# 54rt1n/shardmerge

Hardware: NVIDIA B200
Metric: merged_params_per_sec (higher is better)
Workload: dtype f32

## Files before the change

### shardmerge_b200/csrc/kernels_fft.cu

```cuda
#include <cstdarg>
#include <mutex>
#include "fft_bodies.cuh"
#include "sm_internal.h"

using namespace smfft;

static thread_local char g_err[512] = "";
void sm_set_error(const char* fmt, ...) {
  va_list ap; va_start(ap, fmt); vsnprintf(g_err, sizeof(g_err), fmt, ap); va_end(ap);
}
extern "C" const char* sm_last_error(void) { return g_err; }
extern "C" int sm_version(void) { return 100; }

struct DeviceExec {
  __device__ __forceinline__ int nthreads() const { return (int)blockDim.x; }
  __device__ __forceinline__ int tid_begin() const { return (int)threadIdx.x; }
  __device__ __forceinline__ int tid_end() const { return (int)threadIdx.x + 1; }
  __device__ __forceinline__ void sync() const { __syncthreads(); }
};

extern __shared__ __align__(128) float2 g_dyn_smem[];

__device__ __forceinline__ double warp_sum(double v) {
#pragma unroll
// ... 875 lines not shown
__device__ __forceinline__ void epilogue_store_eo_fast(const RowInvArgs& a, float scale, uint2 bb, uint2* out64, float4* of, int m, pf va,
                                                       pf vb, float& bad) {
  const pf n = pf_bcast(a.inv_n);
  const pf x0 = vb * n, x1 = va * n;
  float y00 = __fmul_rn(pf_lo(x0), scale), y01 = __fmul_rn(pf_hi(x0), scale), y10 = __fmul_rn(pf_lo(x1), scale), y11 = __fmul_rn(pf_hi(x1), scale);
  if (a.out_mode == 0) {
    y00 = __fadd_rn(bf16_bits_to_f32(bb.x & 0xffffu), y00); y10 = __fadd_rn(bits_f32(bb.x & 0xffff0000u), y10);
    y01 = __fadd_rn(bf16_bits_to_f32(bb.y & 0xffffu), y01); y11 = __fadd_rn(bits_f32(bb.y & 0xffff0000u), y11);
    out64[m] = make_uint2(pack_bf16x2_rne(y00, y10), pack_bf16x2_rne(y01, y11));
  } else {
    of[m] = make_float4(y00, y10, y01, y11);
  }
  bad = fmax3_nan(fmax3_nan(bad, fabsf(y00), fabsf(y01)), fabsf(y10), fabsf(y11));
}

__device__ __forceinline__ void epilogue_store_eo(const RowInvArgs& a, float scale, uint2 bb, uint2* out64, float4* of, int m, pf va, pf vb);
struct RowTangleStagedEO {
  const float* re; const float* im; const cf* twC; int H;
  __device__ __forceinline__ void tangle(int k, float& ore, float& oim) const {
    float xr = re[k], xi = im[k], mr = re[2 * H - k], mi = im[2 * H - k];
    if (k == 0) { xi = 0.f; mi = 0.f; }
    const float Ar = xr + mr, Ai = xi - mi, Br = xr - mr, Bi = xi + mi;
    const cf w = ldg_cf(twC + k);
    const float br = Br * w.x + Bi * w.y, bi = Bi * w.x - Br * w.y;
    ore = Ai + br; oim = Ar - bi;
  }
  __device__ __forceinline__ void load(int n, pf& ore, pf& oim) const {
    float u1r, u1i, u2r, u2i;
    tangle(n, u1r, u1i);
    tangle(n + H, u2r, u2i);
    float dr = u1r - u2r, di = u1i - u2i;
    const cf w = ldg_cf(twC + 2 * n);
    cmul(dr, di, w.x, w.y);
    ore = pf_make(u1r + u2r, dr); oim = pf_make(u1i + u2i, di);
  }
};

template <int R1, int R2, int R3, int T, bool kEO>
__global__ void __launch_bounds__(T, 3) k_row2_inv(int R, int C, int P, const __grid_constant__ RowInvArgs a,
                                                   const cf* __restrict__ twC, const cf* __restrict__ twQ, int work_bytes) {
  sm_pdl_enter();
  constexpr int CH = R1 * R2 * R3;
  constexpr int S3 = CH / R3;
  constexpr int kRows = kEO ? 1 : 2;
  constexpr int kTw = kEO ? 4 : 2;
  static_assert(CH / R1 == T && CH / R2 == T && S3 == 2 * T, "k_row2_inv: one butterfly per thread in stages 1-2, two in stage 3");
  __shared__ uint64_t full;
  RowSmem2 sm{reinterpret_cast<ulonglong2*>(g_dyn_smem)};
  char* st_re = reinterpret_cast<char*>(g_dyn_smem) + work_bytes;
  const uint32_t plane_bytes = 4u * (uint32_t)P * kRows;
  char* st_im = st_re + plane_bytes;
  const int tid = threadIdx.x;
  const int npairs = kEO ? R : (R >> 1);
  if (tid == 0) { mbar_init(&full, 1); mbar_fence_init(); }
  __syncthreads();
  const float* im_plane = (a.sel != nullptr && *a.sel != 0) ? a.im_alt : a.im;
  auto prefetch = [&](int pair) {
    if (tid == 0 && pair < npairs) {
      mbar_expect_tx(&full, 2u * plane_bytes);
      bulk_g2s(st_re, a.re + (size_t)pair * kRows * P, plane_bytes, &full);
      bulk_g2s(st_im, im_plane + (size_t)pair * kRows * P, plane_bytes, &full);
    }
  };
  prefetch((int)blockIdx.x);
  const float scale = a.scale_ptr ? *a.scale_ptr : a.scale_host;
  uint32_t phase = 0;
  const int p2 = tid / R1, q2 = tid - p2 * R1;
  const int obase2 = q2 + R1 * R2 * p2, tstep2 = R1 * p2 * kTw;
  for (int pair = blockIdx.x; pair < npairs; pair += gridDim.x) {
    {
      float wr[R1], wi[R1];
      quad_twiddles<R1>(twQ, tid, wr, wi, kEO ? 2 : 1);
      constexpr int Nr = CH / R1;
      pf re[R1], im[R1];
      if constexpr (kEO) {
        mbar_wait(&full, phase); phase ^= 1u;
        RowTangleStagedEO src{reinterpret_cast<const float*>(st_re), reinterpret_cast<const float*>(st_im), twC, CH};
#pragma unroll
        for (int j = 0; j < R1; ++j) src.load(tid + j * Nr, re[j], im[j]);
      } else {
        cf wt[R1];
#pragma unroll
        for (int j = 0; j < R1; ++j) wt[j] = ldg_cf(twC + tid + j * Nr);
        mbar_wait(&full, phase); phase ^= 1u;
        RowTangleStaged2 src{reinterpret_cast<const float*>(st_re), reinterpret_cast<const float*>(st_im), P, CH};
#pragma unroll
        for (int j = 0; j < R1; ++j) src.load(tid + j * Nr, wt[j], re[j], im[j]);
      }
      Dft<R1>::run(re, im);
      sm.store(R1 * tid, re[0], im[0]);
#pragma unroll
      for (int k = 1; k < R1; ++k) {
        pf xr = re[k], xi = im[k];
        cmul(xr, xi, wr[k], wi[k]);
        sm.store(R1 * tid + k, xr, xi);
      }
    }
    __syncthreads();
    prefetch(pair + (int)gridDim.x);
    {
      cf w[R2];
#pragma unroll
      for (int k = 1; k < R2; ++k) w[k] = ldg_cf(twC + tstep2 * k);
      pf re[R2], im[R2];
      constexpr int Nr = CH / R2;
#pragma unroll
      for (int j = 0; j < R2; ++j) sm.load(tid + j * Nr, re[j], im[j]);
      __syncthreads();
      Dft<R2>::run(re, im);
      sm.store(obase2, re[0], im[0]);
#pragma unroll
      for (int k = 1; k < R2; ++k) {
        pf xr = re[k], xi = im[k];
        cmul(xr, xi, w[k].x, w[k].y);
        sm.store(obase2 + k * R1, xr, xi);
      }
    }
    __syncthreads();
    if constexpr (kEO) {
      const uint2* base64 = reinterpret_cast<const uint2*>(a.base + (size_t)pair * C);
      uint2* out64 = a.out_mode == 0 ? reinterpret_cast<uint2*>(a.out_bf16 + (size_t)pair * C) : nullptr;
      float4* of = a.out_mode != 0 ? reinterpret_cast<float4*>(a.out_f32 + (size_t)pair * C) : nullptr;
#pragma unroll
      for (int h = 0; h < 2; ++h) {
        const int b = tid + h * T;
        uint2 bb[R3];
#pragma unroll
        for (int k = 0; k < R3; ++k) bb[k] = a.out_mode == 0 ? __ldg(base64 + b + k * S3) : make_uint2(0u, 0u);
        pf re[R3], im[R3];
#pragma unroll
        for (int j = 0; j < R3; ++j) sm.load(b + j * S3, re[j], im[j]);
        if (h == 1) __syncthreads();
        Dft<R3>::run(re, im);
        float bad = 0.f;
#pragma unroll
        for (int k = 0; k < R3; ++k) epilogue_store_eo_fast(a, scale, bb[k], out64, of, b + k * S3, re[k], im[k], bad);
        if (not_finite(bad)) {
#pragma unroll
          for (int k = 0; k < R3; ++k) epilogue_store_eo(a, scale, bb[k], out64, of, b + k * S3, re[k], im[k]);
        }
      }
    } else {
      const size_t row0 = (size_t)pair * 2;
      const uint32_t* base0 = reinterpret_cast<const uint32_t*>(a.base + row0 * C);
      const uint32_t* base1 = base0 + C / 2;
      uint32_t* out0 = a.out_mode == 0 ? reinterpret_cast<uint32_t*>(a.out_bf16 + row0 * C) : nullptr;
      uint32_t* out1 = out0 + C / 2;
      float* of0 = a.out_mode != 0 ? a.out_f32 + row0 * C : nullptr;
      float* of1 = of0 + C;
#pragma unroll
      for (int h = 0; h < 2; ++h) {
        const int b = tid + h * T;
        uint32_t bb0[R3], bb1[R3];
#pragma unroll
        for (int k = 0; k < R3; ++k) {
          bb0[k] = a.out_mode == 0 ? ldg_u32(base0 + b + k * S3) : 0u;
          bb1[k] = a.out_mode == 0 ? ldg_u32(base1 + b + k * S3) : 0u;
        }
        pf re[R3], im[R3];
#pragma unroll
        for (int j = 0; j < R3; ++j) sm.load(b + j * S3, re[j], im[j]);
        if (h == 1) __syncthreads();
        Dft<R3>::run(re, im);
        float bad = 0.f;
#pragma unroll
        for (int k = 0; k < R3; ++k) epilogue_store2_fast(a, scale, bb0[k], bb1[k], out0, out1, of0, of1, b + k * S3, re[k], im[k], bad);
        if (not_finite(bad)) {
#pragma unroll
          for (int k = 0; k < R3; ++k) epilogue_store2(a, scale, bb0[k], bb1[k], out0, out1, of0, of1, b + k * S3, re[k], im[k]);
        }
      }
    }
  }
}

struct RowTangleGlobal2 {
  const float* re; const float* im; const cf* twC; int P; int Ch;
  __device__ __forceinline__ void load(int k, pf& ore, pf& oim) const {
    pf xr = pf_make(ldg_f32(re + k), ldg_f32(re + P + k)), xi = pf_make(ldg_f32(im + k), ldg_f32(im + P + k));
    pf mr = pf_make(ldg_f32(re + Ch - k), ldg_f32(re + P + Ch - k)), mi = pf_make(ldg_f32(im + Ch - k), ldg_f32(im + P + Ch - k));
    const cf w = ldg_cf(twC + k);
    if (k == 0) { xi = pf_make(0.f, 0.f); mi = xi; }
    const pf Ar = xr + mr, Ai = xi - mi, Br = xr - mr, Bi = xi + mi;
    const pf wx = pf_bcast(w.x), wy = pf_bcast(w.y);
    const pf br = pf_fma(Br, wx, Bi * wy);
    const pf bi = pf_fma(Bi, wx, zero_of(Br) - Br * wy);
    const pf zr = Ar - bi, zi = Ai + br;
    ore = zi; oim = zr;
  }
};

template <int R1, int R2, int R3, int R4, int T, int kCtas>
__global__ void __launch_bounds__(T, kCtas) k_row2_inv4(int R, int C, int P, const __grid_constant__ RowInvArgs a,
                                                    const cf* __restrict__ twC, const cf* __restrict__ twQ) {
  sm_pdl_enter();
  constexpr int CH = R1 * R2 * R3 * R4;
  constexpr int NB1 = CH / R1, NB2 = CH / R2, NB3 = CH / R3, S4 = CH / R4;
  constexpr int s2 = R1, s3 = R1 * R2;
  constexpr int H2 = NB2 / T;
  static_assert(NB2 == H2 * T && H2 >= 1 && H2 <= 2 && NB3 == 2 * T && S4 == 2 * T, "k_row2_inv4: 1-2 / 2 / 2 butterflies per thread in stages 2 / 3 / 4");
  RowSmem2X<true> sm{reinterpret_cast<ulonglong2*>(g_dyn_smem)};
  const int tid = threadIdx.x;
  const int npairs = R >> 1;
  const float* im_plane = (a.sel != nullptr && *a.sel != 0) ? a.im_alt : a.im;
  const float scale = a.scale_ptr ? *a.scale_ptr : a.scale_host;
  auto prefetch = [&](int pair) {
    if (tid == 0 && pair < npairs) {
      bulk_prefetch_l2(a.re + (size_t)pair * 2 * P, 8u * (uint32_t)P);
      bulk_prefetch_l2(im_plane + (size_t)pair * 2 * P, 8u * (uint32_t)P);
      if (a.out_mode == 0) bulk_prefetch_l2(a.base + (size_t)pair * 2 * C, 4u * (uint32_t)C);
    }
  };
  prefetch((int)blockIdx.x);
  for (int pair = blockIdx.x; pair < npairs; pair += gridDim.x) {
    {
      RowTangleGlobal2 src{a.re + (size_t)pair * 2 * P, im_plane + (size_t)pair * 2 * P, twC, P, CH};
#pragma unroll 1
      for (int b = tid; b < NB1; b += T) stockham_bfly_first<R1, pf>(b, CH, twQ, src, sm);
    }
    __syncthreads();
    prefetch(pair + (int)gridDim.x);
    {
      pf re[H2][R2], im[H2][R2];
#pragma unroll
      for (int h = 0; h < H2; ++h)
#pragma unroll
        for (int j = 0; j < R2; ++j) sm.load(tid + h * T + j * NB2, re[h][j], im[h][j]);
      __syncthreads();
#pragma unroll
      for (int h = 0; h < H2; ++h) {
        Dft<R2>::run(re[h], im[h]);
        const int b = tid + h * T;
        const int p = b / s2, q = b - p * s2;
        const int obase = q + s2 * R2 * p, tstep = s2 * p * 2;
        sm.store(obase, re[h][0], im[h][0]);
#pragma unroll
        for (int k = 1; k < R2; ++k) {
          const cf w = ldg_cf(twC + tstep * k);
          pf xr = re[h][k], xi = im[h][k];
          cmul(xr, xi, w.x, w.y);
          sm.store(obase + k * s2, xr, xi);
        }
      }
    }
    __syncthreads();
    {
      pf re[2][R3], im[2][R3];
#pragma unroll
      for (int h = 0; h < 2; ++h)
#pragma unroll
        for (int j = 0; j < R3; ++j) sm.load(tid + h * T + j * NB3, re[h][j], im[h][j]);
      __syncthreads();
#pragma unroll
      for (int h = 0; h < 2; ++h) {
        Dft<R3>::run(re[h], im[h]);
        const int b = tid + h * T;
        const int p = b / s3, q = b - p * s3;
        const int obase = q + s3 * R3 * p, tstep = s3 * p * 2;
        sm.store(obase, re[h][0], im[h][0]);
#pragma unroll
        for (int k = 1; k < R3; ++k) {
          const cf w = ldg_cf(twC + tstep * k);
          pf xr = re[h][k], xi = im[h][k];
          cmul(xr, xi, w.x, w.y);
          sm.store(obase + k * s3, xr, xi);
        }
      }
    }
    __syncthreads();
    {
      const size_t row0 = (size_t)pair * 2;
      const uint32_t* base0 = reinterpret_cast<const uint32_t*>(a.base + row0 * C);
      const uint32_t* base1 = base0 + C / 2;
      uint32_t* out0 = a.out_mode == 0 ? reinterpret_cast<uint32_t*>(a.out_bf16 + row0 * C) : nullptr;
      uint32_t* out1 = out0 + C / 2;
      float* of0 = a.out_mode != 0 ? a.out_f32 + row0 * C : nullptr;
      float* of1 = of0 + C;
#pragma unroll
      for (int h = 0; h < 2; ++h) {
        const int b = tid + h * T;
        uint32_t bb0[R4], bb1[R4];
#pragma unroll
        for (int k = 0; k < R4; ++k) {
          bb0[k] = a.out_mode == 0 ? ldg_u32(base0 + b + k * S4) : 0u;
          bb1[k] = a.out_mode == 0 ? ldg_u32(base1 + b + k * S4) : 0u;
        }
        pf re[R4], im[R4];
#pragma unroll
        for (int j = 0; j < R4; ++j) sm.load(b + j * S4, re[j], im[j]);
        if (h == 1) __syncthreads();
        Dft<R4>::run(re, im);
        float bad = 0.f;
#pragma unroll
        for (int k = 0; k < R4; ++k) epilogue_store2_fast(a, scale, bb0[k], bb1[k], out0, out1, of0, of1, b + k * S4, re[k], im[k], bad);
        if (not_finite(bad)) {
#pragma unroll
          for (int k = 0; k < R4; ++k) epilogue_store2(a, scale, bb0[k], bb1[k], out0, out1, of0, of1, b + k * S4, re[k], im[k]);
        }
      }
    }
  }
}

struct RowTangleGlobalEO {
  const float* re; const float* im; const cf* twC; int H;
  __device__ __forceinline__ void tangle(int k, float& ore, float& oim) const {
    float xr = ldg_f32(re + k), xi = ldg_f32(im + k), mr = ldg_f32(re + 2 * H - k), mi = ldg_f32(im + 2 * H - k);
    if (k == 0) { xi = 0.f; mi = 0.f; }
    const float Ar = xr + mr, Ai = xi - mi, Br = xr - mr, Bi = xi + mi;
    const cf w = ldg_cf(twC + k);
    const float br = Br * w.x + Bi * w.y, bi = Bi * w.x - Br * w.y;
    ore = Ai + br; oim = Ar - bi;
  }
  __device__ __forceinline__ void load(int n, pf& ore, pf& oim) const {
    float u1r, u1i, u2r, u2i;
    tangle(n, u1r, u1i);
    tangle(n + H, u2r, u2i);
    float dr = u1r - u2r, di = u1i - u2i;
    const cf w = ldg_cf(twC + 2 * n);
    cmul(dr, di, w.x, w.y);
    ore = pf_make(u1r + u2r, dr); oim = pf_make(u1i + u2i, di);
  }
};

__device__ __forceinline__ void epilogue_store_eo(const RowInvArgs& a, float scale, uint2 bb, uint2* out64, float4* of, int m, pf va, pf vb) {
  const pf n = pf_bcast(a.inv_n);
  const pf x0 = vb * n, x1 = va * n;
  const float x00 = pf_lo(x0), x01 = pf_hi(x0), x10 = pf_lo(x1), x11 = pf_hi(x1);
  const bool add_base = a.out_mode == 0;
  const float b00 = add_base ? bf16_bits_to_f32(bb.x & 0xffffu) : 0.f, b10 = add_base ? bits_f32(bb.x & 0xffff0000u) : 0.f;
  const float b01 = add_base ? bf16_bits_to_f32(bb.y & 0xffffu) : 0.f, b11 = add_base ? bits_f32(bb.y & 0xffff0000u) : 0.f;
  float y00, y01, y10, y11;
  epi_finish4(a, scale, add_base, x00, x01, x10, x11, b00, b01, b10, b11, y00, y01, y10, y11);
  if (add_base) out64[m] = make_uint2(pack_bf16x2_rne(y00, y10), pack_bf16x2_rne(y01, y11));
  else of[m] = make_float4(y00, y10, y01, y11);
}

template <int R1, int R2, int R3, int R4, int T, int kCtas>
__global__ void __launch_bounds__(T, kCtas) k_row1_inv_eo(int R, int C, int P, const __grid_constant__ RowInvArgs a,
                                                      const cf* __restrict__ twC, const cf* __restrict__ twQ2) {
  sm_pdl_enter();
  constexpr int CH = R1 * R2 * R3 * R4;
  constexpr int NB1 = CH / R1, NB2 = CH / R2, NB3 = CH / R3, S4 = CH / R4;
  constexpr int s2 = R1, s3 = R1 * R2;
  constexpr int H2 = NB2 / T;
  static_assert(NB2 == H2 * T && H2 >= 1 && H2 <= 2 && NB3 == 2 * T && S4 == 2 * T, "k_row1_inv_eo: 1-2 / 2 / 2 butterflies per thread in stages 2 / 3 / 4");
  RowSmem2X<false> sm{reinterpret_cast<ulonglong2*>(g_dyn_smem)};
  const int tid = threadIdx.x;
  const float* im_plane = (a.sel != nullptr && *a.sel != 0) ? a.im_alt : a.im;
  const float scale = a.scale_ptr ? *a.scale_ptr : a.scale_host;
  auto prefetch = [&](int row) {
    if (tid == 0 && row < R) {
      bulk_prefetch_l2(a.re + (size_t)row * P, 4u * (uint32_t)P);
      bulk_prefetch_l2(im_plane + (size_t)row * P, 4u * (uint32_t)P);
      if (a.out_mode == 0) bulk_prefetch_l2(a.base + (size_t)row * C, 2u * (uint32_t)C);
    }
  };
  prefetch((int)blockIdx.x);
  for (int row = blockIdx.x; row < R; row += gridDim.x) {
    {
      RowTangleGlobalEO src{a.re + (size_t)row * P, im_plane + (size_t)row * P, twC, CH};
#pragma unroll 1
      for (int b = tid; b < NB1; b += T) stockham_bfly_first<R1, pf>(b, CH, twQ2, src, sm, 2);
    }
    __syncthreads();
    prefetch(row + (int)gridDim.x);
    {
      pf re[H2][R2], im[H2][R2];
#pragma unroll
      for (int h = 0; h < H2; ++h)
#pragma unroll
        for (int j = 0; j < R2; ++j) sm.load(tid + h * T + j * NB2, re[h][j], im[h][j]);
      __syncthreads();
#pragma unroll
      for (int h = 0; h < H2; ++h) {
        Dft<R2>::run(re[h], im[h]);
        const int b = tid + h * T;
        const int p = b / s2, q = b - p * s2;
        const int obase = q + s2 * R2 * p, tstep = s2 * p * 4;
        sm.store(obase, re[h][0], im[h][0]);
#pragma unroll
        for (int k = 1; k < R2; ++k) {
          const cf w = ldg_cf(twC + tstep * k);
          pf xr = re[h][k], xi = im[h][k];
          cmul(xr, xi, w.x, w.y);
          sm.store(obase + k * s2, xr, xi);
        }
      }
    }
    __syncthreads();
    {
      pf re[2][R3], im[2][R3];
#pragma unroll
      for (int h = 0; h < 2; ++h)
#pragma unroll
        for (int j = 0; j < R3; ++j) sm.load(tid + h * T + j * NB3, re[h][j], im[h][j]);
      __syncthreads();
#pragma unroll
      for (int h = 0; h < 2; ++h) {
        Dft<R3>::run(re[h], im[h]);
        const int b = tid + h * T;
        const int p = b / s3, q = b - p * s3;
        const int obase = q + s3 * R3 * p, tstep = s3 * p * 4;
        sm.store(obase, re[h][0], im[h][0]);
#pragma unroll
        for (int k = 1; k < R3; ++k) {
          const cf w = ldg_cf(twC + tstep * k);
          pf xr = re[h][k], xi = im[h][k];
          cmul(xr, xi, w.x, w.y);
          sm.store(obase + k * s3, xr, xi);
        }
      }
    }
    __syncthreads();
    {
      const uint2* base64 = reinterpret_cast<const uint2*>(a.base + (size_t)row * C);
      uint2* out64 = a.out_mode == 0 ? reinterpret_cast<uint2*>(a.out_bf16 + (size_t)row * C) : nullptr;
      float4* of = a.out_mode != 0 ? reinterpret_cast<float4*>(a.out_f32 + (size_t)row * C) : nullptr;
#pragma unroll
      for (int h = 0; h < 2; ++h) {
        const int b = tid + h * T;
        uint2 bb[R4];
#pragma unroll
        for (int k = 0; k < R4; ++k) bb[k] = a.out_mode == 0 ? __ldg(base64 + b + k * S4) : make_uint2(0u, 0u);
        pf re[R4], im[R4];
#pragma unroll
        for (int j = 0; j < R4; ++j) sm.load(b + j * S4, re[j], im[j]);
        if (h == 1) __syncthreads();
        Dft<R4>::run(re, im);
        float bad = 0.f;
#pragma unroll
        for (int k = 0; k < R4; ++k) epilogue_store_eo_fast(a, scale, bb[k], out64, of, b + k * S4, re[k], im[k], bad);
        if (not_finite(bad)) {
#pragma unroll
          for (int k = 0; k < R4; ++k) epilogue_store_eo(a, scale, bb[k], out64, of, b + k * S4, re[k], im[k]);
        }
      }
    }
  }
}

__global__ void k_scale_row(float* re, float* im, int n, const float* scale_dev, float scale_host, int write_im) {
  sm_pdl_enter();
  const float s = scale_dev ? *scale_dev : scale_host;
  for (int i = blockIdx.x * blockDim.x + threadIdx.x; i < n; i += gridDim.x * blockDim.x) {
    re[i] *= s;
    if (write_im) im[i] *= s;
  }
}

__global__ void k_init_twiddles(cf* tw, int M) {
  for (int j = blockIdx.x * blockDim.x + threadIdx.x; j < M; j += gridDim.x * blockDim.x) {
    double s, c;
    sincospi(2.0 * (double)j / (double)M, &s, &c);
    cf w; w.x = (float)c; w.y = (float)(-s);
    tw[j] = w;
  }
}

__global__ void k_init_quads(cf* quad, int n_b, int N) {
  for (int i = blockIdx.x * blockDim.x + threadIdx.x; i < 4 * n_b; i += gridDim.x * blockDim.x) {
    const long long e = ((long long)(i >> 2) << (i & 3)) % N;
    double s, c;
    sincospi(2.0 * (double)e / (double)N, &s, &c);
    cf w; w.x = (float)c; w.y = (float)(-s);
    quad[i] = w;
  }
}

__global__ void k_inv_norm(const double* sumsq, float* out) {
  sm_pdl_enter();
  const double ss = *sumsq;
  const float nrm = (float)sqrt(ss);
  *out = (nrm != 0.f) ? (1.0f / nrm) : 1.0f;
}

static std::once_flag g_attr_once;
static int g_attr_rc = 0;
static int ensure_attrs() {
  std::call_once(g_attr_once, [] {
    int dev = 0, optin = 0;
    cudaError_t e = cudaGetDevice(&dev);
    if (e == cudaSuccess) e = cudaDeviceGetAttribute(&optin, cudaDevAttrMaxSharedMemoryPerBlockOptin, dev);
    auto set = [&](const void* fn) {
      cudaFuncAttributes fa;
      if (e == cudaSuccess) e = cudaFuncGetAttributes(&fa, fn);
      if (e == cudaSuccess)
        e = cudaFuncSetAttribute(fn, cudaFuncAttributeMaxDynamicSharedMemorySize, optin - (int)fa.sharedSizeBytes);
    };
    set((const void*)k_row_fwd);
    set((const void*)k_row_inv);
    set((const void*)k_col);
    if (e != cudaSuccess) { sm_set_error("shared-memory opt-in failed: %s", cudaGetErrorString(e)); g_attr_rc = -100; }
  });
  return g_attr_rc;
}

extern "C" sm_plan* sm_plan_create(int R, int C) {
  sm_plan* pl = new sm_plan;
  int rc = sm_make_plan(R, C, &pl->p);
  if (rc != 0) {
    sm_set_error("unsupported tensor shape [%d][%d] for the sm_100a FFT (rc=%d): C must be even, the prime factors of "
                 "C/2 and R at most %d, and R = a * b with one a-point and one b-point column instance of 32 columns "
                 "each fitting in shared memory", R, C, rc, SM_GENERIC_MAX);
    delete pl;
    return nullptr;
  }
  return pl;
}
extern "C" void sm_plan_destroy(sm_plan* plan) { delete plan; }
extern "C" int sm_plan_pitch(const sm_plan* plan) { return plan->p.P; }
extern "C" int sm_plan_col_passes(const sm_plan* plan) { return plan->p.col_passes; }
extern "C" int sm_plan_col_launches(const sm_plan* plan) {
  return plan->p.col_passes == 2 ? 2 : 1;
}
extern "C" int sm_plan_row_freq(const sm_plan* plan, int stored) { return sm_row_freq(&plan->p, stored); }
extern "C" size_t sm_plan_table_bytes(const sm_plan* plan) {
  return sm_tab_bytes(plan->p);
}
extern "C" int sm_plan_describe(const sm_plan* plan, char* buf, int buflen) {
  const SmPlan& p = plan->p;
  int n = snprintf(buf, buflen, "R=%d C=%d P=%d row[%d thr, smem %d/%d, pad %d]:", p.R, p.C, p.P,
                   p.row_threads, p.row_smem_fwd, p.row_smem_inv, p.row_pad);
  for (int i = 0; i < p.n_row && n < buflen; ++i) n += snprintf(buf + n, buflen - n, " %d", p.row_rad[i]);
  if (n < buflen) n += snprintf(buf + n, buflen - n, " | col passes=%d Ra=%d[%d thr]:", p.col_passes, p.Ra, p.thrA);
  for (int i = 0; i < p.nA && n < buflen; ++i) n += snprintf(buf + n, buflen - n, " %d", p.radA[i]);
  if (p.col_passes == 2) {
    if (n < buflen) n += snprintf(buf + n, buflen - n, " Rb=%d[%d thr]:", p.Rb, p.thrB);
    for (int i = 0; i < p.nB && n < buflen; ++i) n += snprintf(buf + n, buflen - n, " %d", p.radB[i]);
  }
  return n;
}

extern "C" int sm_plan_init_tables(const sm_plan* plan, void* tables, void* stream) {
  const SmPlan& p = plan->p;
  cudaStream_t st = (cudaStream_t)stream;
  cf* twC = reinterpret_cast<cf*>(tables);
  cf* twR = reinterpret_cast<cf*>(reinterpret_cast<char*>(tables) + sm_tab_off_R(p));
  k_init_twiddles<<<(p.C + 255) / 256, 256, 0, st>>>(twC, p.C);
  SM_LAUNCH_CHECK();
  k_init_twiddles<<<(p.R + 255) / 256, 256, 0, st>>>(twR, p.R);
  SM_LAUNCH_CHECK();
  cf* twQ = reinterpret_cast<cf*>(reinterpret_cast<char*>(tables) + sm_tab_off_Q(p));
  const int nq = sm_quad_count(p);
  if (nq > 0) {
    k_init_quads<<<(4 * nq + 255) / 256, 256, 0, st>>>(twQ, nq, p.Ch);
    SM_LAUNCH_CHECK();
  }
  return 0;
}

static const cf* tabC(const SmPlan&, const void* tables) { return reinterpret_cast<const cf*>(tables); }
static const cf* tabQ(const SmPlan& p, const void* tables) {
  return reinterpret_cast<const cf*>(reinterpret_cast<const char*>(tables) + sm_tab_off_Q(p));
}
static const cf* tabR(const SmPlan& p, const void* tables) {
  return reinterpret_cast<const cf*>(reinterpret_cast<const char*>(tables) + sm_tab_off_R(p));
}

static int g_optin_smem = 0;
template <class K>
static cudaError_t opt_in(K kernel, bool* done) {
  if (*done) return cudaSuccess;
  if (g_optin_smem == 0) {
    int dev = 0;
    cudaError_t e = cudaGetDevice(&dev);
    if (e == cudaSuccess) e = cudaDeviceGetAttribute(&g_optin_smem, cudaDevAttrMaxSharedMemoryPerBlockOptin, dev);
    if (e != cudaSuccess) return e;
  }
  cudaFuncAttributes fa;
  cudaError_t e = cudaFuncGetAttributes(&fa, (const void*)kernel);
  if (e == cudaSuccess)
    e = cudaFuncSetAttribute((const void*)kernel, cudaFuncAttributeMaxDynamicSharedMemorySize,
                             g_optin_smem - (int)fa.sharedSizeBytes);
  if (e == cudaSuccess) *done = true;
  return e;
}

template <int R1, int R2, int NW>
static int launch_col_p(bool inverse, bool big_tw, dim3 grid, const ColCtArgs& a, const cf* twR, cudaStream_t st) {
  static bool done[4] = {false, false, false, false};
  const int smem = (R2 > 1) ? R1 * R2 * SM_COL_TILE * 8 : 0;
  cudaError_t e;
#define SM_COLP_CASE(INV, BIG, IDX)                                                       \
  e = opt_in(k_col_p<R1, R2, NW, INV, BIG>, &done[IDX]);                                  \
  if (e != cudaSuccess) { sm_set_error("opt_in: %s", cudaGetErrorString(e)); return -100; } \
  sm_launch(k_col_p<R1, R2, NW, INV, BIG>, dim3(grid), dim3(NW * 32), (size_t)(smem), st, a, twR);
  if (!inverse && big_tw) { SM_COLP_CASE(false, true, 0) }
  else if (!inverse) { SM_COLP_CASE(false, false, 1) }
  else if (big_tw) { SM_COLP_CASE(true, true, 2) }
  else { SM_COLP_CASE(true, false, 3) }
#undef SM_COLP_CASE
  SM_LAUNCH_CHECK();
  return 0;
}

template <int R1, int R2, int R3, int NW>
static int launch_col_p3(bool inverse, bool big_tw, dim3 grid, const ColCtArgs& a, const cf* twR, cudaStream_t st) {
  static bool done[4] = {false, false, false, false};
  const int smem = R1 * R2 * R3 * SM_COL_TILE * 8;
  cudaError_t e;
#define SM_COLP3_CASE(INV, BIG, IDX)                                                      \
  e = opt_in(k_col_p3<R1, R2, R3, NW, INV, BIG>, &done[IDX]);                             \
  if (e != cudaSuccess) { sm_set_error("opt_in: %s", cudaGetErrorString(e)); return -100; } \
  sm_launch(k_col_p3<R1, R2, R3, NW, INV, BIG>, dim3(grid), dim3(NW * 32), (size_t)(smem), st, a, twR);
  if (!inverse && big_tw) { SM_COLP3_CASE(false, true, 0) }
  else if (!inverse) { SM_COLP3_CASE(false, false, 1) }
  else if (big_tw) { SM_COLP3_CASE(true, true, 2) }
  else { SM_COLP3_CASE(true, false, 3) }
#undef SM_COLP3_CASE
  SM_LAUNCH_CHECK();
  return 0;
}

static int try_col_p(int n_rad, const int* rad, bool inverse, bool big_tw, dim3 grid, const ColCtArgs& a,
                     const cf* twR, cudaStream_t st) {
  if (n_rad != 2) return 1;
  const int r1 = rad[0], r2 = rad[1];
  if (r1 == 8 && r2 == 8) return launch_col_p<8, 8, 4>(inverse, big_tw, grid, a, twR, st);
  if (r1 == 16 && r2 == 8) return launch_col_p3<8, 8, 2, 8>(inverse, big_tw, grid, a, twR, st);
  if (r1 == 7 && r2 == 16) return launch_col_p3<7, 8, 2, 8>(inverse, big_tw, grid, a, twR, st);
  if (r1 == 16 && r2 == 16) return launch_col_p<16, 16, 8>(inverse, big_tw, grid, a, twR, st);
  if (r1 == 11 && r2 == 8) return launch_col_p<11, 8, 4>(inverse, big_tw, grid, a, twR, st);
  if (r1 == 8 && r2 == 4) return launch_col_p<8, 4, 2>(inverse, big_tw, grid, a, twR, st);
  return 1;
}

static int g_num_sms = 0;
static int num_sms() {
  if (g_num_sms == 0) {
    int dev = 0;
    if (cudaGetDevice(&dev) != cudaSuccess || cudaDeviceGetAttribute(&g_num_sms, cudaDevAttrMultiProcessorCount, dev) != cudaSuccess)
      g_num_sms = 148;
  }
  return g_num_sms;
}
template <int R1, int R2, int R3, int R4, int T, bool kPad>
static int try_row2_fwd(const SmPlan& p, const RowFwdArgs& fa, const cf* twC, const cf* twQ, double* sumsq, cudaStream_t st) {
  if constexpr (R4 == 1 && kPad && (R1 * R2 * R3) / R3 == 2 * T && (R1 * R2 * R3) / R1 == T && (R1 * R2 * R3) / R2 == T) {
    constexpr int CH = R1 * R2 * R3;
    if (fa.mode != 0 || (p.R & 1) || p.R < 2 || p.C % 8 != 0) return 1;
    static bool done = false;
    static int occ = 0;
    const int work_bytes = ((CH + (CH >> 4) + 1) * 16 + 127) / 128 * 128;
    const int smem = work_bytes + 8 * p.C;
    if (smem > 227 * 1024 - 256) return 1;
    cudaError_t e = opt_in(k_row2_fwd<R1, R2, R3, T, false>, &done);
    if (e == cudaSuccess && occ == 0) e = cudaOccupancyMaxActiveBlocksPerMultiprocessor(&occ, k_row2_fwd<R1, R2, R3, T, false>, T, smem);
    if (e != cudaSuccess) { sm_set_error("row2 setup: %s", cudaGetErrorString(e)); return -100; }
    int grid = num_sms() * (occ > 0 ? occ : 1);
    if (grid > p.R / 2) grid = p.R / 2;
    sm_launch(k_row2_fwd<R1, R2, R3, T, false>, dim3(grid), dim3(T), (size_t)(smem), st, p.R, p.C, p.P, fa, twC, twQ, sumsq, work_bytes, RowFwdPair{});
    SM_LAUNCH_CHECK();
    return 0;
  } else {
    return 1;
  }
}

template <int R1, int R2, int R3, int R4, int T, int kCtas>
static int launch_row2_fwd4(const SmPlan& p, const RowFwdArgs& fa, const cf* twC, const cf* twQ, double* sumsq, cudaStream_t st) {
  constexpr int CH = R1 * R2 * R3 * R4;
  if (fa.mode != 0 || (p.R & 1) || p.R < 2 || p.C % 8 != 0 || p.Ch != CH) return 1;
  static bool done = false;
  const int smem = (CH + (CH >> 3) + 1) * 16;
  if (smem > 227 * 1024 - 256) return 1;
  cudaError_t e = opt_in(k_row2_fwd4<R1, R2, R3, R4, T, kCtas>, &done);
  if (e != cudaSuccess) { sm_set_error("row2 fwd4 setup: %s", cudaGetErrorString(e)); return -100; }
  int grid = num_sms() * kCtas;
  if (grid > p.R / 2) grid = p.R / 2;
  sm_launch(k_row2_fwd4<R1, R2, R3, R4, T, kCtas>, dim3(grid), dim3(T), (size_t)(smem), st, p.R, p.C, p.P, fa, twC, twQ, sumsq);
  SM_LAUNCH_CHECK();
  return 0;
}

template <int R1, int R2, int R3, int R4, int T, int kCtas>
static int launch_row2_inv4(const SmPlan& p, const RowInvArgs& ia, const cf* twC, const cf* twQ, cudaStream_t st) {
  constexpr int CH = R1 * R2 * R3 * R4;
  if (ia.cull_thr != nullptr || (p.R & 1) || p.R < 2 || p.C % 8 != 0 || p.P % 4 != 0 || p.Ch != CH) return 1;
  static bool done = false;
  const int smem = (CH + (CH >> 3) + 1) * 16;
  if (smem > 227 * 1024 - 256) return 1;
  cudaError_t e = opt_in(k_row2_inv4<R1, R2, R3, R4, T, kCtas>, &done);
  if (e != cudaSuccess) { sm_set_error("row2 inv4 setup: %s", cudaGetErrorString(e)); return -100; }
  int grid = num_sms() * kCtas;
  if (grid > p.R / 2) grid = p.R / 2;
  sm_launch(k_row2_inv4<R1, R2, R3, R4, T, kCtas>, dim3(grid), dim3(T), (size_t)(smem), st, p.R, p.C, p.P, ia, twC, twQ);
  SM_LAUNCH_CHECK();
  return 0;
}

template <int R1, int R2, int R3, int R4, int T, int kCtas, bool kPair = false>
static int launch_row1_fwd_eo(const SmPlan& p, const RowFwdArgs& fa, const cf* twC, const cf* twQ, double* sumsq, cudaStream_t st,
                              const RowFwdPair& pr = RowFwdPair{}) {
  constexpr int CH = R1 * R2 * R3 * R4;
  if (fa.mode != 0 || p.R < 1 || p.C % 8 != 0 || p.Ch != 2 * CH) return 1;
  static bool done = false;
  const int smem = CH * 16;
  cudaError_t e = opt_in(k_row1_fwd_eo<R1, R2, R3, R4, T, kCtas, kPair>, &done);
  if (e != cudaSuccess) { sm_set_error("row1 fwd eo setup: %s", cudaGetErrorString(e)); return -100; }
  int grid = num_sms() * kCtas;
  if (grid > p.R) grid = p.R;
  sm_launch(k_row1_fwd_eo<R1, R2, R3, R4, T, kCtas, kPair>, dim3(grid), dim3(T), (size_t)(smem), st, p.R, p.C, p.P, fa, twC, twQ, sumsq, pr);
  SM_LAUNCH_CHECK();
  return 0;
}

template <int R1, int R2, int R3, int T>
static int launch_row1_fwd_eo3(const SmPlan& p, const RowFwdArgs& fa, const cf* twC, const cf* twQ, double* sumsq, cudaStream_t st) {
  constexpr int CH = R1 * R2 * R3;
  if (fa.mode != 0 || p.R < 2 || p.C % 8 != 0 || p.Ch != 2 * CH) return 1;
  static bool done = false;
  static int occ = 0;
  const int work_bytes = ((CH + (CH >> 4) + 1) * 16 + 127) / 128 * 128;
  const int smem = work_bytes + 4 * p.C;
  cudaError_t e = opt_in(k_row2_fwd<R1, R2, R3, T, true>, &done);
  if (e == cudaSuccess && occ == 0) e = cudaOccupancyMaxActiveBlocksPerMultiprocessor(&occ, k_row2_fwd<R1, R2, R3, T, true>, T, smem);
  if (e != cudaSuccess) { sm_set_error("row1 fwd eo3 setup: %s", cudaGetErrorString(e)); return -100; }
  int grid = num_sms() * (occ > 0 ? occ : 1);
  if (grid > p.R) grid = p.R;
  sm_launch(k_row2_fwd<R1, R2, R3, T, true>, dim3(grid), dim3(T), (size_t)(smem), st, p.R, p.C, p.P, fa, twC, twQ, sumsq, work_bytes, RowFwdPair{});
  SM_LAUNCH_CHECK();
  return 0;
}

static int try_row2_fwd4(const SmPlan& p, const RowFwdArgs& fa, const cf* twC, const cf* twQ, double* sumsq, cudaStream_t st) {
  if (p.Ch == 4096) return launch_row1_fwd_eo3<16, 16, 8, 128>(p, fa, twC, twQ, sumsq, st);
  if (p.Ch == 14336) return launch_row1_fwd_eo<7, 16, 8, 8, 448, 1>(p, fa, twC, twQ, sumsq, st);
  if (p.Ch == 7168) return launch_row1_fwd_eo<7, 8, 8, 8, 224, 2>(p, fa, twC, twQ, sumsq, st);
  if (p.Ch == 1024) return launch_row2_fwd4<8, 8, 4, 4, 128, 4>(p, fa, twC, twQ, sumsq, st);
  if (p.Ch == 2816) return launch_row1_fwd_eo<11, 8, 4, 4, 176, 2>(p, fa, twC, twQ, sumsq, st);
  return 1;
}
template <int R1, int R2, int R3, int R4, int T, int kCtas>
static int launch_row1_inv_eo(const SmPlan& p, const RowInvArgs& ia, const cf* twC, const cf* twQ, cudaStream_t st) {
  constexpr int CH = R1 * R2 * R3 * R4;
  if (ia.cull_thr != nullptr || p.R < 1 || p.C % 8 != 0 || p.Ch != 2 * CH) return 1;
  static bool done = false;
  const int smem = CH * 16;
  cudaError_t e = opt_in(k_row1_inv_eo<R1, R2, R3, R4, T, kCtas>, &done);
  if (e != cudaSuccess) { sm_set_error("row1 inv eo setup: %s", cudaGetErrorString(e)); return -100; }
  int grid = num_sms() * kCtas;
  if (grid > p.R) grid = p.R;
  sm_launch(k_row1_inv_eo<R1, R2, R3, R4, T, kCtas>, dim3(grid), dim3(T), (size_t)(smem), st, p.R, p.C, p.P, ia, twC, twQ);
  SM_LAUNCH_CHECK();
  return 0;
}

template <int R1, int R2, int R3, int T>
static int launch_row1_inv_eo3(const SmPlan& p, const RowInvArgs& ia, const cf* twC, const cf* twQ, cudaStream_t st) {
  constexpr int CH = R1 * R2 * R3;
  if (ia.cull_thr != nullptr || p.R < 2 || p.C % 8 != 0 || p.P % 4 != 0 || p.Ch != 2 * CH) return 1;
  static bool done = false;
  static int occ = 0;
  const int work_bytes = ((CH + (CH >> 4) + 1) * 16 + 127) / 128 * 128;
  const int smem = work_bytes + 8 * p.P;
  cudaError_t e = opt_in(k_row2_inv<R1, R2, R3, T, true>, &done);
  if (e == cudaSuccess && occ == 0) e = cudaOccupancyMaxActiveBlocksPerMultiprocessor(&occ, k_row2_inv<R1, R2, R3, T, true>, T, smem);
  if (e != cudaSuccess) { sm_set_error("row1 inv eo3 setup: %s", cudaGetErrorString(e)); return -100; }
  int grid = num_sms() * (occ > 0 ? occ : 1);
  if (grid > p.R) grid = p.R;
  sm_launch(k_row2_inv<R1, R2, R3, T, true>, dim3(grid), dim3(T), (size_t)(smem), st, p.R, p.C, p.P, ia, twC, twQ, work_bytes);
  SM_LAUNCH_CHECK();
  return 0;
}

static int try_row2_inv4(const SmPlan& p, const RowInvArgs& ia, const cf* twC, const cf* twQ, cudaStream_t st) {
  if (p.Ch == 4096) return launch_row1_inv_eo3<16, 16, 8, 128>(p, ia, twC, twQ, st);
  if (p.Ch == 14336) return launch_row1_inv_eo<7, 16, 8, 8, 448, 1>(p, ia, twC, twQ, st);
  if (p.Ch == 7168) return launch_row1_inv_eo<7, 8, 8, 8, 224, 2>(p, ia, twC, twQ, st);
  if (p.Ch == 1024) return launch_row2_inv4<8, 8, 4, 4, 128, 4>(p, ia, twC, twQ, st);
  if (p.Ch == 2816) return launch_row1_inv_eo<11, 8, 4, 4, 176, 2>(p, ia, twC, twQ, st);
  return 1;
}

template <int R1, int R2, int R3, int R4, int T, bool kPad>
static int try_row2_inv(const SmPlan& p, const RowInvArgs& ia, const cf* twC, const cf* twQ, cudaStream_t st) {
  if constexpr (R4 == 1 && kPad && (R1 * R2 * R3) / R3 == 2 * T && (R1 * R2 * R3) / R1 == T && (R1 * R2 * R3) / R2 == T) {
    constexpr int CH = R1 * R2 * R3;
    if (ia.cull_thr != nullptr || (p.R & 1) || p.R < 2 || p.C % 8 != 0 || p.P % 4 != 0) return 1;
    static bool done = false;
    static int occ = 0;
    const int work_bytes = ((CH + (CH >> 4) + 1) * 16 + 127) / 128 * 128;
    const int smem = work_bytes + 16 * p.P;
    if (smem > 227 * 1024 - 256) return 1;
    cudaError_t e = opt_in(k_row2_inv<R1, R2, R3, T, false>, &done);
    if (e == cudaSuccess && occ == 0) e = cudaOccupancyMaxActiveBlocksPerMultiprocessor(&occ, k_row2_inv<R1, R2, R3, T, false>, T, smem);
    if (e != cudaSuccess) { sm_set_error("row2 inv setup: %s", cudaGetErrorString(e)); return -100; }
    int grid = num_sms() * (occ > 0 ? occ : 1);
    if (grid > p.R / 2) grid = p.R / 2;
    sm_launch(k_row2_inv<R1, R2, R3, T, false>, dim3(grid), dim3(T), (size_t)(smem), st, p.R, p.C, p.P, ia, twC, twQ, work_bytes);
    SM_LAUNCH_CHECK();
    return 0;
  } else {
    return 1;
  }
}

template <int R1, int R2, int R3, int R4, int T, bool kPad>
static int launch_row_ct(bool inverse, const SmPlan& p, const RowFwdArgs* fa, const RowInvArgs* ia, const cf* twC,
                         const cf* twQ, double* sumsq, cudaStream_t st) {
  static bool done[4] = {false, false, false, false};
  static int occ[2] = {0, 0};
  constexpr int CH = R1 * R2 * R3 * R4;
  if (!inverse) {
    int rc = try_row2_fwd<R1, R2, R3, R4, T, kPad>(p, *fa, twC, twQ, sumsq, st);
    if (rc <= 0) return rc;
    rc = try_row2_fwd4(p, *fa, twC, twQ, sumsq, st);
    if (rc <= 0) return rc;
  }
  if (inverse) {
    int rc = try_row2_inv<R1, R2, R3, R4, T, kPad>(p, *ia, twC, twQ, st);
    if (rc <= 0) return rc;
    rc = try_row2_inv4(p, *ia, twC, twQ, st);
    if (rc <= 0) return rc;
  }
  constexpr int nst = (R2 > 1) + (R3 > 1) + (R4 > 1) + 1;
  constexpr int bufstride = kPad ? (CH + (CH >> 4) + 1) : CH;
  cudaError_t e;
  const int work_bytes = (((!inverse ? (nst >= 2 ? 2 : 1) : (nst >= 3 ? 2 : 1)) * bufstride * 8) + 127) / 128 * 128;
  const int stage_bytes = !inverse ? 4 * p.C : 8 * p.P + ((ia->out_mode == 0) ? 2 * p.C : 0);
  const bool aligned = (p.C % 8 == 0);
  if (aligned && work_bytes + stage_bytes <= 227 * 1024 - 256 && p.R >= 2) {
    const int smem = work_bytes + stage_bytes;
    const int which = inverse ? 1 : 0;
    if (!inverse) {
      e = opt_in(k_row_fwd_tma<R1, R2, R3, R4, T, kPad>, &done[2]);
      if (e == cudaSuccess && occ[0] == 0)
        e = cudaOccupancyMaxActiveBlocksPerMultiprocessor(&occ[0], k_row_fwd_tma<R1, R2, R3, R4, T, kPad>, T, smem);
    } else {
      e = opt_in(k_row_inv_tma<R1, R2, R3, R4, T, kPad>, &done[3]);
      if (e == cudaSuccess && occ[1] == 0)
        e = cudaOccupancyMaxActiveBlocksPerMultiprocessor(&occ[1], k_row_inv_tma<R1, R2, R3, R4, T, kPad>, T, smem);
    }
    if (e != cudaSuccess) { sm_set_error("row tma setup: %s", cudaGetErrorString(e)); return -100; }
    int grid = num_sms() * (occ[which] > 0 ? occ[which] : 1);
    if (grid > p.R) grid = p.R;
    if (!inverse) sm_launch(k_row_fwd_tma<R1, R2, R3, R4, T, kPad>, dim3(grid), dim3(T), (size_t)(smem), st, p.R, p.C, p.P, *fa, twC, twQ, sumsq, work_bytes);
    else sm_launch(k_row_inv_tma<R1, R2, R3, R4, T, kPad>, dim3(grid), dim3(T), (size_t)(smem), st, p.R, p.C, p.P, *ia, twC, twQ, work_bytes);
    SM_LAUNCH_CHECK();
    return 0;
  }
  if (!inverse) {
    e = opt_in(k_row_fwd_ct<R1, R2, R3, R4, T, kPad>, &done[0]);
    if (e != cudaSuccess) { sm_set_error("opt_in: %s", cudaGetErrorString(e)); return -100; }
    sm_launch(k_row_fwd_ct<R1, R2, R3, R4, T, kPad>, dim3(p.R), dim3(T), (size_t)(p.row_smem_fwd), st, p.C, p.P, *fa, twC, twQ, sumsq);
  } else {
    e = opt_in(k_row_inv_ct<R1, R2, R3, R4, T, kPad>, &done[1]);
    if (e != cudaSuccess) { sm_set_error("opt_in: %s", cudaGetErrorString(e)); return -100; }
    sm_launch(k_row_inv_ct<R1, R2, R3, R4, T, kPad>, dim3(p.R), dim3(T), (size_t)(p.row_smem_inv), st, p.C, p.P, *ia, twC, twQ);
  }
  SM_LAUNCH_CHECK();
  return 0;
}

static bool row_radices_are(const SmPlan& p, int n, int a, int b, int c, int d) {
  if (p.n_row != n) return false;
  const int want[4] = {a, b, c, d};
  for (int i = 0; i < n; ++i) if (p.row_rad[i] != want[i]) return false;
  return true;
}

static int try_row_ct(bool inverse, const SmPlan& p, const RowFwdArgs* fa, const RowInvArgs* ia, const cf* twC,
                      const cf* twQ, double* sumsq, cudaStream_t st) {
  auto is = [&](int n, int a, int b, int c, int d) { return row_radices_are(p, n, a, b, c, d); };
  if (is(3, 16, 8, 8, 1) && p.row_threads == 64 && p.row_pad) return launch_row_ct<16, 8, 8, 1, 64, true>(inverse, p, fa, ia, twC, twQ, sumsq, st);
  if (is(3, 16, 16, 8, 1) && p.row_threads == 128 && p.row_pad) return launch_row_ct<16, 16, 8, 1, 128, true>(inverse, p, fa, ia, twC, twQ, sumsq, st);
  if (is(3, 16, 16, 16, 1) && p.row_threads == 256 && p.row_pad) return launch_row_ct<16, 16, 16, 1, 256, true>(inverse, p, fa, ia, twC, twQ, sumsq, st);
  if (is(3, 11, 16, 16, 1) && p.row_threads == 192 && p.row_pad) return launch_row_ct<11, 16, 16, 1, 192, true>(inverse, p, fa, ia, twC, twQ, sumsq, st);
  if (is(4, 7, 16, 8, 8) && p.row_threads == 448 && p.row_pad) return launch_row_ct<7, 16, 8, 8, 448, true>(inverse, p, fa, ia, twC, twQ, sumsq, st);
  if (is(4, 7, 16, 16, 8) && p.row_threads == 512 && !p.row_pad) return launch_row_ct<7, 16, 16, 8, 512, false>(inverse, p, fa, ia, twC, twQ, sumsq, st);
  return 1;
}

static int launch_row_fwd(const SmPlan& p, const void* tables, const RowFwdArgs& a, double* sumsq, cudaStream_t st) {
  if (ensure_attrs()) return -100;
  {
    const int rc = try_row_ct(false, p, &a, nullptr, tabC(p, tables), tabQ(p, tables), sumsq, st);
    if (rc <= 0) return rc;
  }
  sm_launch(k_row_fwd, dim3(p.R), dim3(p.row_threads), (size_t)(p.row_smem_fwd), st, p, a, tabC(p, tables), tabQ(p, tables), sumsq);
  SM_LAUNCH_CHECK();
  return 0;
}

extern "C" int sm_fwd_rows_bf16(const sm_plan* plan, const void* tables, const void* base_bf16, const void* ft_bf16,
                                float* re, float* im, double* sumsq, void* stream) {
  RowFwdArgs a{};
  a.mode = 0; a.base = (const uint16_t*)base_bf16; a.ft = (const uint16_t*)ft_bf16;
  a.m1 = 1.f; a.m2 = 1.f; a.re = re; a.im = im;
  return launch_row_fwd(plan->p, tables, a, sumsq, (cudaStream_t)stream);
}

enum RowPairKind { kRowPairNone = 0, kRowPairRow2, kRowPairEo7168 };
static RowPairKind row_pair_kind(const SmPlan& p) {
  if (p.C % 8 != 0 || p.R < 1) return kRowPairNone;
  if (row_radices_are(p, 3, 16, 16, 8, 1) && p.row_threads == 128 && p.row_pad && p.R % 2 == 0) return kRowPairRow2;
  if (row_radices_are(p, 4, 7, 16, 8, 8) && p.row_threads == 448 && p.row_pad && p.Ch == 7168) return kRowPairEo7168;
  return kRowPairNone;
}

template <int R1, int R2, int R3, int T>
static int launch_row2_fwd_pair(const SmPlan& p, const RowFwdArgs& fa, const RowFwdPair& pr, const cf* twC, const cf* twQ,
                                double* sumsq, cudaStream_t st) {
  constexpr int CH = R1 * R2 * R3;
  static bool done = false;
  static int occ = 0;
  const int work_bytes = ((CH + (CH >> 4) + 1) * 16 + 127) / 128 * 128;
  const int smem = work_bytes + 6 * p.C;
  cudaError_t e = opt_in(k_row2_fwd<R1, R2, R3, T, false, true>, &done);
  if (e == cudaSuccess && occ == 0) e = cudaOccupancyMaxActiveBlocksPerMultiprocessor(&occ, k_row2_fwd<R1, R2, R3, T, false, true>, T, smem);
  if (e != cudaSuccess) { sm_set_error("row2 pair setup: %s", cudaGetErrorString(e)); return -100; }
  int grid = num_sms() * (occ > 0 ? occ : 1);
  if (grid > p.R) grid = p.R;
  sm_launch(k_row2_fwd<R1, R2, R3, T, false, true>, dim3(grid), dim3(T), (size_t)(smem), st, p.R, p.C, p.P, fa, twC, twQ, sumsq, work_bytes, pr);
  SM_LAUNCH_CHECK();
  return 0;
}

extern "C" int sm_fwd_rows_pair_supported(const sm_plan* plan) { return row_pair_kind(plan->p) != kRowPairNone ? 1 : 0; }

extern "C" int sm_fwd_rows_bf16_pair(const sm_plan* plan, const void* tables, const void* base_bf16, const void* ft0_bf16,
                                     const void* ft1_bf16, float* re0, float* im0, float* re1, float* im1, void* ctl,
                                     double target_norm_offset, double target_norm, void* stream) {
  const SmPlan& p = plan->p;
  RowFwdArgs a{};
  a.mode = 0; a.base = (const uint16_t*)base_bf16; a.ft = (const uint16_t*)ft0_bf16;
  a.m1 = 1.f; a.m2 = 1.f; a.re = re0; a.im = im0;
  const RowFwdPair pr{(const uint16_t*)ft1_bf16, re1, im1, (unsigned char*)ctl, target_norm_offset, target_norm};
  double* sumsq = reinterpret_cast<double*>((unsigned char*)ctl + SM_CTL_SUMSQ);
  const cf* twC = tabC(p, tables);
  const cf* twQ = tabQ(p, tables);
  cudaStream_t st = (cudaStream_t)stream;
  switch (row_pair_kind(p)) {
    case kRowPairRow2: return launch_row2_fwd_pair<16, 16, 8, 128>(p, a, pr, twC, twQ, sumsq, st);
    case kRowPairEo7168: return launch_row1_fwd_eo<7, 8, 8, 8, 224, 2, true>(p, a, twC, twQ, sumsq, st, pr);
    default: break;
  }
  sm_set_error("sm_fwd_rows_bf16_pair: no paired row kernel for [%d][%d] (sm_fwd_rows_pair_supported)", p.R, p.C);
  return -102;
}

extern "C" int sm_fwd_rows_f32(const sm_plan* plan, const void* tables, const float* x, float m1, float m2,
                               float* re, float* im, double* sumsq, void* stream) {
  RowFwdArgs a{};
  a.mode = 1; a.x32 = x; a.m1 = m1; a.m2 = m2; a.re = re; a.im = im;
  return launch_row_fwd(plan->p, tables, a, sumsq, (cudaStream_t)stream);
}

static int launch_col(const SmPlan& p, const void* tables, int sweep, int inverse, float* re, float* im,
                      const float* cull_thr, const float* scale_dev, float scale_host, int use_scale,
                      int write_im, cudaStream_t st, float* im_alt = nullptr, const int* sel = nullptr,
                      const int* wsel = nullptr, int wskip = 0) {
  if (ensure_attrs()) return -100;
  ColArgs ca{};
  int n_inst = 0;
  sm_col_args(p, sweep, inverse, &ca, &n_inst);
  ca.re = re; ca.im = im; ca.cull_thr = cull_thr; ca.im_alt = im_alt; ca.sel = sel;
  ca.scale_ptr = scale_dev; ca.scale_host = scale_host; ca.use_scale = use_scale;
  ca.write_im = write_im; ca.wsel = wsel; ca.wskip = wskip;
  const int ntiles = sm_col_tiles(p);
  {
    ColCtArgs c{};
    c.p0 = inverse ? im : re; c.p1 = inverse ? re : im;
    c.p0_alt = inverse ? im_alt : nullptr; c.sel = inverse ? sel : nullptr;
    c.P = p.P; c.Ch = p.Ch; c.inst_mul = ca.inst_mul; c.elem_mul = ca.elem_mul; c.tw_mul = ca.tw_mul;
    c.thr_ptr = cull_thr; c.scale_ptr = use_scale ? scale_dev : nullptr;
    c.scale = use_scale ? scale_host : 1.0f; c.write_p1_fwd = write_im; c.wsel = wsel; c.wskip = wskip;
    const int rc = try_col_p(ca.n_rad, ca.rad, inverse != 0, ca.big_tw != 0, dim3(ntiles, n_inst), c, tabR(p, tables), st);
    if (rc <= 0) return rc;
  }
  const int threads = (sweep == 0) ? p.thrA : p.thrB;
  const int smem = (sweep == 0) ? p.smemA : p.smemB;
  sm_launch(k_col, dim3(dim3(ntiles, n_inst)), dim3(threads), (size_t)(smem), st, p, ca, tabR(p, tables));
  SM_LAUNCH_CHECK();
  return 0;
}

extern "C" int sm_fwd_cols(const sm_plan* plan, const void* tables, float* re, float* im,
                           const float* scale_dev, float scale_host, int write_im, void* stream) {
  return sm_fwd_cols_sel(plan, tables, re, im, scale_dev, scale_host, write_im, nullptr, 0, stream);
}

int sm_fwd_cols_sel(const sm_plan* plan, const void* tables, float* re, float* im, const float* scale_dev, float scale_host,
                    int write_im, const int* wsel, int wskip, void* stream) {
  const SmPlan& p = plan->p;
  cudaStream_t st = (cudaStream_t)stream;
  if (p.col_passes == 0) {
    sm_launch(k_scale_row, dim3((p.Ch + 1 + 255) / 256), dim3(256), (size_t)(0), st, re, im, p.Ch + 1, scale_dev, scale_host, write_im);
    SM_LAUNCH_CHECK();
    return 0;
  }
  for (int sweep = 0; sweep < p.col_passes; ++sweep) {
    const bool lastsweep = (sweep == p.col_passes - 1);
    int rc = launch_col(p, tables, sweep, 0, re, im, nullptr, scale_dev, scale_host, lastsweep ? 1 : 0,
                        lastsweep ? write_im : 1, st, nullptr, nullptr, lastsweep ? wsel : nullptr, wskip);
    if (rc) return rc;
  }
  return 0;
}

extern "C" int sm_inv_norm(const double* sumsq, float* out, void* stream) {
  sm_launch(k_inv_norm, dim3(1), dim3(1), (size_t)(0), (cudaStream_t)stream, sumsq, out);
  SM_LAUNCH_CHECK();
  return 0;
}

int sm_inv_cols_sel(const sm_plan* plan, const void* tables, float* re, float* im, float* im_alt, const int* sel,
                    const float* cull_thr, void* stream) {
  const SmPlan& p = plan->p;
  for (int i = 0; i < p.col_passes; ++i) {
    const int sweep = p.col_passes - 1 - i;
    int rc = launch_col(p, tables, sweep, 1, re, im, i == 0 ? cull_thr : nullptr, nullptr, 1.f, 0, 1,
                        (cudaStream_t)stream, im_alt, sel);
    if (rc) return rc;
  }
  return 0;
}

extern "C" int sm_inv_cols(const sm_plan* plan, const void* tables, float* re, float* im, const float* cull_thr,
                           void* stream) {
  return sm_inv_cols_sel(plan, tables, re, im, nullptr, nullptr, cull_thr, stream);
}

static int launch_row_inv(const SmPlan& p, const void* tables, RowInvArgs& a, cudaStream_t st) {
  if (ensure_attrs()) return -100;
  a.inv_n = (float)(1.0 / ((double)p.R * (double)p.C));
  if (p.col_passes != 0) a.cull_thr = nullptr;
  {
    const int rc = try_row_ct(true, p, nullptr, &a, tabC(p, tables), tabQ(p, tables), nullptr, st);
    if (rc <= 0) return rc;
  }
  sm_launch(k_row_inv, dim3(p.R), dim3(p.row_threads), (size_t)(p.row_smem_inv), st, p, a, tabC(p, tables), tabQ(p, tables));
  SM_LAUNCH_CHECK();
  return 0;
}

int sm_inv_rows_bf16_sel(const sm_plan* plan, const void* tables, const float* re, const float* im,
                         const float* im_alt, const int* sel, const float* cull_thr, const void* base_bf16,
                         void* out_bf16, const float* scale_dev, float scale_host, int check_ifft, uint32_t* flags4,
                         void* stream) {
  RowInvArgs a{};
// ... 39 lines not shown
```

Baseline: 54.87 billion.

## Stage inverse EO row inputs into shared memory via TMA bulk copy with mbarrier

The inverse even/odd row kernel used to prefetch each row's real and imaginary planes into L2 and then gather them with scattered global loads in the first FFT stage. It now issues bulk global-to-shared copies for the next row, tracked by an mbarrier, and the first stage reads from a shared staging buffer instead. This is meant to cut the latency and L2 traffic of the mirrored global gathers. In exchange it needs 8*P more bytes of dynamic shared memory per CTA and adds a P%4 requirement, which may reduce occupancy or send some shapes to a fallback path.

```diff
diff --git a/shardmerge_b200/csrc/kernels_fft.cu b/shardmerge_b200/csrc/kernels_fft.cu
--- a/shardmerge_b200/csrc/kernels_fft.cu
+++ b/shardmerge_b200/csrc/kernels_fft.cu
@@ -1201,26 +1201,6 @@
   }
 }
 
-struct RowTangleGlobalEO {
-  const float* re; const float* im; const cf* twC; int H;
-  __device__ __forceinline__ void tangle(int k, float& ore, float& oim) const {
-    float xr = ldg_f32(re + k), xi = ldg_f32(im + k), mr = ldg_f32(re + 2 * H - k), mi = ldg_f32(im + 2 * H - k);
-    if (k == 0) { xi = 0.f; mi = 0.f; }
-    const float Ar = xr + mr, Ai = xi - mi, Br = xr - mr, Bi = xi + mi;
-    const cf w = ldg_cf(twC + k);
-    const float br = Br * w.x + Bi * w.y, bi = Bi * w.x - Br * w.y;
-    ore = Ai + br; oim = Ar - bi;
-  }
-  __device__ __forceinline__ void load(int n, pf& ore, pf& oim) const {
-    float u1r, u1i, u2r, u2i;
-    tangle(n, u1r, u1i);
-    tangle(n + H, u2r, u2i);
-    float dr = u1r - u2r, di = u1i - u2i;
-    const cf w = ldg_cf(twC + 2 * n);
-    cmul(dr, di, w.x, w.y);
-    ore = pf_make(u1r + u2r, dr); oim = pf_make(u1i + u2i, di);
-  }
-};
 
 __device__ __forceinline__ void epilogue_store_eo(const RowInvArgs& a, float scale, uint2 bb, uint2* out64, float4* of, int m, pf va, pf vb) {
   const pf n = pf_bcast(a.inv_n);
@@ -1244,21 +1224,29 @@
   constexpr int s2 = R1, s3 = R1 * R2;
   constexpr int H2 = NB2 / T;
   static_assert(NB2 == H2 * T && H2 >= 1 && H2 <= 2 && NB3 == 2 * T && S4 == 2 * T, "k_row1_inv_eo: 1-2 / 2 / 2 butterflies per thread in stages 2 / 3 / 4");
+  __shared__ uint64_t full;
   RowSmem2X<false> sm{reinterpret_cast<ulonglong2*>(g_dyn_smem)};
+  const float* st_re = reinterpret_cast<const float*>(reinterpret_cast<const char*>(g_dyn_smem) + CH * 16);
+  const float* st_im = st_re + P;
   const int tid = threadIdx.x;
+  if (tid == 0) { mbar_init(&full, 1); mbar_fence_init(); }
+  __syncthreads();
   const float* im_plane = (a.sel != nullptr && *a.sel != 0) ? a.im_alt : a.im;
   const float scale = a.scale_ptr ? *a.scale_ptr : a.scale_host;
   auto prefetch = [&](int row) {
     if (tid == 0 && row < R) {
-      bulk_prefetch_l2(a.re + (size_t)row * P, 4u * (uint32_t)P);
-      bulk_prefetch_l2(im_plane + (size_t)row * P, 4u * (uint32_t)P);
+      mbar_expect_tx(&full, 8u * (uint32_t)P);
+      bulk_g2s((void*)st_re, a.re + (size_t)row * P, 4u * (uint32_t)P, &full);
+      bulk_g2s((void*)st_im, im_plane + (size_t)row * P, 4u * (uint32_t)P, &full);
       if (a.out_mode == 0) bulk_prefetch_l2(a.base + (size_t)row * C, 2u * (uint32_t)C);
     }
   };
   prefetch((int)blockIdx.x);
+  uint32_t phase = 0;
   for (int row = blockIdx.x; row < R; row += gridDim.x) {
     {
-      RowTangleGlobalEO src{a.re + (size_t)row * P, im_plane + (size_t)row * P, twC, CH};
+      mbar_wait(&full, phase); phase ^= 1u;
+      RowTangleStagedEO src{st_re, st_im, twC, CH};
 #pragma unroll 1
       for (int b = tid; b < NB1; b += T) stockham_bfly_first<R1, pf>(b, CH, twQ2, src, sm, 2);
     }
@@ -1634,9 +1622,10 @@
 template <int R1, int R2, int R3, int R4, int T, int kCtas>
 static int launch_row1_inv_eo(const SmPlan& p, const RowInvArgs& ia, const cf* twC, const cf* twQ, cudaStream_t st) {
   constexpr int CH = R1 * R2 * R3 * R4;
-  if (ia.cull_thr != nullptr || p.R < 1 || p.C % 8 != 0 || p.Ch != 2 * CH) return 1;
+  if (ia.cull_thr != nullptr || p.R < 1 || p.C % 8 != 0 || p.P % 4 != 0 || p.Ch != 2 * CH) return 1;
   static bool done = false;
-  const int smem = CH * 16;
+  const int smem = CH * 16 + 8 * p.P;
+  if (smem > 227 * 1024 - 256) return 1;
   cudaError_t e = opt_in(k_row1_inv_eo<R1, R2, R3, R4, T, kCtas>, &done);
   if (e != cudaSuccess) { sm_set_error("row1 inv eo setup: %s", cudaGetErrorString(e)); return -100; }
   int grid = num_sms() * kCtas;
```

Result: no change. 55.00 billion, median of 6 (+0.2%).
